# ChrisTho23/DrakeGPT

Hardware: AMD Instinct MI355X
Metric: training tokens/sec (fwd+bwd+AdamW) (higher is better)
Workload: dtype bf16; 1 GPU; TransformerLM_scaled: V=80 C=384 T=256 heads=6 layers=6 dropout=0.2; fwd+bwd+AdamW; hipGraph=on; batch_per_gpu=64, global_batch=64, seq_len=256, parallelism=dp1, dp_gradient_buckets=1, params=10800464

## Files before the change

### drakegpt_amd/_lib.py

```python
from __future__ import annotations

import ctypes as C
import os

import torch

_HERE = os.path.dirname(os.path.abspath(__file__))
LIB_PATH = os.path.join(_HERE, "lib", "libdrakegpt_hip.so")

DG_F32 = 0
DG_BF16 = 1
DG_FP8_E4M3 = 2
DG_FP8_E5M2 = 3
DG_F32X3 = 4
ABI_VERSION = 21


class GemmNtArgs(C.Structure):
    _fields_ = [
        ("A", C.c_void_p), ("lda", C.c_int64),
        ("B", C.c_void_p), ("ldb", C.c_int64),
        ("C", C.c_void_p), ("ldc", C.c_int64),
        ("M", C.c_int32), ("N", C.c_int32), ("K", C.c_int32),
        ("in_dtype", C.c_int32), ("out_dtype", C.c_int32),
# ... 81 lines not shown
    "dg_layernorm_bwd": [_vp, _i, _vp, _vp, _vp, _vp, _vp, _vp, _vp, _vp, _i64, _i, _i, _i, _vp],
    "dg_layernorm_bwd_fused": [_vp, _i, _vp, _vp, _vp, _vp, _vp, _vp, _i, _vp, _vp, _i64, _i, _i, _i, _vp, _i, _f, _vp, _u32, _vp, _vp],
    "dg_layernorm_bwd_fused_fp8": [_vp, _i, _vp, _vp, _vp, _vp, _vp, _vp, _i, _vp, _vp, _i64, _i, _i, _i, _vp, _f, _vp, _u32, _vp, _vp, _vp, _vp, _vp, _i, _vp],
    "dg_gemm_nt": [C.POINTER(GemmNtArgs), _vp],
    "dg_gemm_nt_sign_bits_supported": [C.POINTER(GemmNtArgs)],
    "dg_gemm_nt_fp8_out_supported": [C.POINTER(GemmNtArgs)],
    "dg_gemm_nt_colsum_supported": [C.POINTER(GemmNtArgs)],
    "dg_gemm_nt_colsum_rows": [C.POINTER(GemmNtArgs)],
    "dg_gemm_nt_sign_bits_bytes": [_i, _i],
    "dg_fp8_amax": [_vp, _i, _i64, _vp, _i, _vp, _vp],
    "dg_fp8_quantize": [_vp, _i, _vp, _i, _i64, _vp, _i, _vp, _vp, _vp],
    "dg_fp8_quantize_delayed": [_vp, _i, _vp, _i, _i64, _vp, _vp, _vp, _vp],
    "dg_gemm_tn": [_vp, _i64, _vp, _i64, _vp, _i64, _i64, _i, _i, _i, _i, _i, _vp],
    "dg_gemm_tn_grouped": [C.POINTER(TnProblem), _i, _i, _vp, _i64, _vp],
    "dg_gemm_tn_grouped_workspace_bytes": [C.POINTER(TnProblem), _i],
    "dg_reduce_partials": [_vp, _i64, _i, _vp, _i64, _vp],
    "dg_colsum": [_vp, _i64, _i, _vp, _i64, _i, _i, _i, _vp],
    "dg_dropout_bwd_cast": [_vp, _i, _i64, _vp, _i64, _i, _i, _i, _f, _vp, _u32, _vp, _i64, _vp, _i64, _i, _vp],
    "dg_cast": [_vp, _i, _vp, _i, _i64, _vp],
    "dg_transpose_cast": [_vp, _i64, _vp, _i64, _i, _i, _i, _vp],
    "dg_transpose_cast_batched": [_vp, _i, _i, _i, _i, _vp],
    "dg_transpose_u8_batched": [_vp, _i, _i, _vp],
    "dg_attn_keep_bits_bytes": [_i, _i, _i, _i, _i],
    "dg_attn_fwd": [_vp, _vp, _vp, _i, _i, _i, _i, _f, _f, _vp, _u32, _i, _vp, _i64, _vp],
    "dg_attn_bwd": [_vp, _vp, _vp, _vp, _vp, _vp, _i64, _i, _i, _i, _i, _f, _f, _vp, _u32, _i, _vp, _i64, _vp],
    "dg_attn_fp8_out_supported": [_i, _i, _i, _i, _i],
    "dg_attn_fwd_fp8": [_vp, _vp, _vp, _i, _i, _i, _i, _f, _f, _vp, _u32, _i, _vp, _i64, C.POINTER(AttnFp8Out), _vp],
    "dg_attn_bwd_fp8": [_vp, _vp, _vp, _vp, _vp, _vp, _i64, _i, _i, _i, _i, _f, _f, _vp, _u32, _i, _vp, _i64, C.POINTER(AttnFp8Out), _vp],
    "dg_attn_bwd_workspace_bytes": [_i, _i, _i, _i, _i],
    "dg_attn_decode": [_vp, _vp, _i, _i, _i, _i, _i, _f, _i, _vp],
    "dg_cross_entropy": [_vp, _i, _i64, _vp, _vp, _vp, _i64, _i, _f, _vp, _i, _i, _vp],
    "dg_cross_entropy_fp8": [_vp, _i64, _vp, _vp, _vp, _i64, _f, _i, _i, _vp, _i64, _vp],
    "dg_cross_entropy_fused": [_vp, _i64, _vp, _vp, _vp, _i64, _i, _f, _i, _i, _vp, _i64, _i, _vp, _vp, _vp, _f, _vp],
    "dg_reduce_sum": [_vp, _i64, _f, _vp, _vp],
    "dg_softmax_rows": [_vp, _i64, _vp, _i64, _i, _i, _vp],
    "dg_adamw_step": [_vp, _vp, _vp, _vp, _i64, _vp, _vp, _f, _vp, _i, _vp],
    "dg_sumsq_parts": [_i64],
    "dg_sumsq_partials": [_vp, _i64, _vp, _vp],
    "dg_grad_norm_finalize": [_vp, _i, _f, _vp, _vp, _vp],
    "dg_adamw_step_clip": [_vp, _vp, _vp, _vp, _i64, _vp, _vp, _f, _vp, _vp, _i, _vp],
    "dg_block_chain_supported": [_i, _i],
    "dg_block_chain_fwd": [C.POINTER(BlockChainArgs), _vp],
    "dg_l2_warm": [_vp, _i64, _vp],
    "dg_pack_chain_weights": [_vp, _i64, _vp, _i, _i, _vp],
    "dg_pack_chain_weights_batched": [_vp, _i, _i, _vp],
    "dg_block_chain_bwd_supported": [_i, _i],
    "dg_block_chain_bwd": [C.POINTER(BlockChainBwdArgs), _vp],
}


def _load() -> C.CDLL:
    if not os.path.exists(LIB_PATH):
        raise RuntimeError(
            f"drakegpt_amd: {LIB_PATH} is missing. Build it with `python -m drakegpt_amd.build` "
            "(needs hipcc; cross-compiles for gfx950 without a GPU). There is no CPU fallback.")
    lib = C.CDLL(LIB_PATH)
    for name, argtypes in SIGNATURES.items():
        try:
            fn = getattr(lib, name)
        except AttributeError as e:
            raise RuntimeError(f"drakegpt_amd: {LIB_PATH} does not export {name}; rebuild it") from e
        fn.argtypes = argtypes
        fn.restype = C.c_int
    lib.dg_gemm_nt_sign_bits_bytes.restype = C.c_int64
    lib.dg_gemm_tn_grouped_workspace_bytes.restype = C.c_int64
    lib.dg_attn_bwd_workspace_bytes.restype = C.c_int64
# ... 18 lines not shown
```

### drakegpt_amd/build.py

```python
from __future__ import annotations

import hashlib
import os
import shutil
import subprocess
import sys
from concurrent.futures import ThreadPoolExecutor

PKG = os.path.dirname(os.path.abspath(__file__))
CSRC = os.path.join(PKG, "csrc")
LIBDIR = os.path.join(PKG, "lib")
OBJDIR = os.environ.get("DRAKEGPT_OBJDIR", os.path.join(os.environ.get("TMPDIR", "/tmp"), f"drakegpt_amd_build_{os.getuid()}"))
LIB = os.path.join(LIBDIR, "libdrakegpt_hip.so")
ARCH = "gfx950"

SOURCES = [
    "elementwise.hip",
    "layernorm.hip",
    "gemm.hip",
    "gemm_fp8.hip",
    "gemm_x3.hip",
    "fp8.hip",
    "attention.hip",
    "attention_simple.hip",
    "attention_mfma.hip",
    "cross_entropy.hip",
    "chain.hip",
    "chain_bwd.hip",
    "grad_clip.hip",
]


def _hipcc() -> str:
    for c in (os.environ.get("HIPCC"), "/opt/rocm/bin/hipcc", shutil.which("hipcc")):
        if c and os.path.exists(c):
            return c
    raise RuntimeError("hipcc not found (looked at $HIPCC, /opt/rocm/bin/hipcc, PATH)")


def _digest(paths) -> str:
    h = hashlib.sha256()
    for p in paths:
        with open(p, "rb") as f:
            h.update(f.read())
    return h.hexdigest()


def build(force: bool = False, save_temps: bool = False, verbose: bool = True) -> str:
    os.makedirs(LIBDIR, exist_ok=True)
    os.makedirs(OBJDIR, exist_ok=True)
    hipcc = _hipcc()
    headers = [os.path.join(CSRC, "common.h"), os.path.join(CSRC, "gemm_nt_ws.h"), os.path.join(PKG, "..", "include", "drakegpt_hip.h")]
    hdr_digest = _digest(headers)
    flags = ["--offload-arch=" + ARCH, "-O3", "-fPIC", "-std=c++17",
             "-Wno-unused-result", "-I", os.path.join(PKG, "..", "include")]
    if save_temps:
        flags += ["-save-temps=obj"]

    def compile_one(src: str):
# ... 41 lines not shown
```

### drakegpt_amd/engine.py

```python
from __future__ import annotations

from typing import Dict, List, Optional, Tuple

import torch

from . import ops
from . import sublayers as S
from .model import TransformerLM
from .optim import check_max_grad_norm

Tensor = torch.Tensor
ALIGN = 64


def _round(n: int, a: int = ALIGN) -> int:
    return (n + a - 1) // a * a


class _Layout:
    def __init__(self):
        self.entries: Dict[str, Tuple[int, Tuple[int, ...]]] = {}
        self.size = 0

    def add(self, key: str, shape) -> int:
# ... 178 lines not shown
        self.chain_bwd = (_os.environ.get("DG_CHAIN_BWD", "0") == "1" and self.chain_full and self.stream_dtype == torch.bfloat16
                          and ops.block_chain_bwd_supported(self.M, self.C, self.act))
        self.chain_ln = (_os.environ.get("DG_CHAIN_LN", "0") == "1" and not self.fp8 and self.NH * self.H == self.C
                         and ops.block_chain_supported(self.M, self.C, self.act))
        self._build_layout()
        self.dp_buckets = self._choose_buckets(self._dp_buckets_arg)
        if self.dp_buckets > 1:
            self.chain_bwd = False
        self._alloc_and_adopt()
        self.hyper = torch.tensor([lr, betas[0], betas[1], eps, weight_decay], dtype=torch.float32, device=self.dev)
        self.max_grad_norm = None if max_grad_norm is None else check_max_grad_norm(max_grad_norm)
        self.clip_state = self.norm_work = self.last_grad_norm = None
        if self.max_grad_norm is not None:
            self.clip_state = torch.tensor([0.0, 1.0, self.max_grad_norm, 0.0], dtype=torch.float32, device=self.dev)
            self.norm_work = ops.grad_norm_workspace([self.gflat], self.dev)
            self.last_grad_norm = self.clip_state[0]
        self.state = ops.new_rng_state(seed + 0x9E3779B97F4A7C15 * rank & 0xFFFFFFFFFFFFFFFF, self.dev, 0)
        self.off_block = torch.zeros((self.OFFSET_ROWS, self.B), dtype=torch.int64, device=self.dev)
        self.offsets = self.off_block[0]
        self.off_ctl = torch.tensor([0, 1], dtype=torch.int32, device=self.dev)
        self._off_rows, self._off_left = 1, None
        self.x = torch.zeros((self.B, self.T), dtype=torch.int64, device=self.dev)
        self.y = torch.zeros((self.B, self.T), dtype=torch.int64, device=self.dev)
        self.loss = torch.zeros((), dtype=torch.float32, device=self.dev)
        self.dl_scale = torch.full((1,), 1.0 / (self.M * 57344.0), dtype=torch.float32, device=self.dev)
        self.loss_scratch = torch.zeros((2048 + 1,), dtype=torch.float32, device=self.dev)
        self.corpus: Optional[Tensor] = None
        self._graphs = None
        self._eval_graph = None
        self.force_dp_path = False
        self.debug_timing = False
        self.last_timing: Optional[dict] = None
        self.keep_logits = False
        self.last_logits: Optional[Tensor] = None
        self.refresh_shadows()

    def _build_layout(self):
        C, V, L, NH, H = self.C, self.V, self.L, self.NH, self.H
        A, Bv, E, Z = _Layout(), _Layout(), _Layout(), _Layout()
        for l in range(L):
            A.add(f"{l}.wqkv", (3 * NH * H, C))
            A.add(f"{l}.wproj", (C, NH * H))
            A.add(f"{l}.w1", (4 * C, C))
            A.add(f"{l}.w2", (C, 4 * C))
        A.add("lm.w", (V, C))
        for l in range(L):
            for k, n in (("bproj", C), ("b1", 4 * C), ("b2", C), ("ln1w", C), ("ln1b", C), ("ln2w", C), ("ln2b", C)):
                Bv.add(f"{l}.{k}", (n,))
        Bv.add("lm.b", (V,))
        E.add("tok", (V, C))
        E.add("pos", (self.model.context_length, C))
        Z.add("lnf.w", (C,))
        Z.add("lnf.b", (C,))
        self.layA, self.layB, self.layE, self.layZ = A, Bv, E, Z
        self.offA, self.offB = 0, A.size
        self.offE = A.size + Bv.size
        self.n_active = self.offE + E.size
        self.offZ = self.n_active
        self.n_total = self.n_active + Z.size

    def _choose_buckets(self, arg: Optional[int]) -> int:
        import os
        if arg is None and os.environ.get("DG_DP_BUCKETS"):
            arg = int(os.environ["DG_DP_BUCKETS"])
        if not self.grouped_dw or (self.world == 1 and arg is None):
            return 1
# ... 252 lines not shown
            kw = dict(o=o, x=x, wproj=pk(P["wproj"]), bproj=P["bproj"], ln2w=P["ln2w"], ln2b=P["ln2b"], w1=pk(P["w1"]), b1=P["b1"],
                      w2=pk(P["w2"]), b2=P["b2"], dropout_p=p, rng_state=run.rng, site_proj=S.site_proj(l), site_ffn=S.site_ffn(l))
            if last:
                r = ops.block_chain_fwd(1, M, C, **kw)
            else:
                Pn = self._layer_params(l + 1)
                r = ops.block_chain_fwd(0, M, C, ln1w=Pn["ln1w"], ln1b=Pn["ln1b"], wqkv=pk(Pn["wqkv"]), **kw)
            if want_grad:
                saved.append(((x, h1, m1, r1, qkv, o, lse), (r["x1"], r["h2"], r["mean2"], r["rstd2"], r["f"], r["bits"])))
            x = r["x2"]
            if not last:
                P, h1, m1, r1, qkv = Pn, r["h1"], r["mean1"], r["rstd1"], r["qkv"]
        return x, saved

    def _head(self, run: S.Run, h: Tensor, y_idx: Optional[Tensor], want_grad: bool, saved, M: int):
        if self.bf16_logits and y_idx is not None and not self.keep_logits:
            buf = torch.empty((M, S.k_pad(self.V, self.act)), dtype=self.act, device=self.dev)
            if self.fp8_head and run.fp8 and h.dtype == torch.bfloat16:
                Wl = self.param_view("lm.w")
                xq, xs = S._quantize_operand(run, h, S.E4M3, "lm.x")
                h.dg_fp8x = (xq, xs)
                wq, ws = self.weights.fwd8(Wl)
                logits = ops.gemm_nt(xq, wq, self.act, scale_a=xs, scale_b=ws, bias=self.param_view("lm.b"), out=buf[:, :self.V])
                if want_grad and M == self.M:
                    q8 = torch.empty((M, buf.shape[1]), dtype=S.E5M2, device=self.dev)
                    rows = ops.cross_entropy_fp8(logits, y_idx.view(M), self.V, buf, 1.0 / M, q8)
                    buf.dg_q8 = (q8, self.dl_scale)
                else:
                    rows = ops.cross_entropy(logits, y_idx.view(M), self.V, dlogits=buf if want_grad else None, grad_scale=1.0 / M)
                return None, rows, (saved, h, buf)
            logits, (xa,) = S.linear_fwd(run, h, self.param_view("lm.w"), self.param_view("lm.b"), out=buf[:, :self.V])
            rows = ops.cross_entropy(logits, y_idx.view(M), self.V, dlogits=buf if want_grad else None, grad_scale=1.0 / M)
            return None, rows, (saved, xa, buf)
        logits, (xa,) = S.linear_fwd(run, h, self.param_view("lm.w"), self.param_view("lm.b"), pad_rows=True)
        if y_idx is None:
            return logits, None, None
        dlogits = None
        if want_grad:
            dlogits = torch.empty((M, S.k_pad(self.V, self.act)), dtype=self.act, device=self.dev)
            if M == self.M and ops.cross_entropy_fused_supported(logits, dlogits, self.G):
                part, stride, n = FlatSink(self).vector("lm.b", self.V)
                rows = ops.cross_entropy_fused(logits, y_idx.view(M), self.V, dlogits, 1.0 / M, part, stride, n, self.loss_scratch,
                                               self.loss, 1.0 / M)
                return logits, rows, (saved, xa, dlogits, True)
        rows = ops.cross_entropy(logits, y_idx.view(M), self.V, dlogits=dlogits, grad_scale=1.0 / M)
        return logits, rows, (saved, xa, dlogits)

    def _backward_begin(self, run: S.Run, x_idx: Tensor, ctx) -> dict:
        saved, xa, dlogits = ctx[:3]
        head_done = len(ctx) > 3
        st = dict(run=run, x_idx=x_idx, saved=saved, sink=FlatSink(self), g_next=None, g0=None)
        g = dlogits[:, :self.V]
        q8 = getattr(dlogits, "dg_q8", None)
        if q8 is not None:
            g.dg_fp8 = (q8[0][:, :self.V], q8[1])
        st["dh"] = S.linear_bwd_from_act(run, (xa,), g, self.param_view("lm.w"), True, st["sink"], {"w": "lm.w", "b": "lm.b"},
                                         bias_done=head_done)
        return st

    def _backward_layers(self, st: dict, layers) -> None:
        run, sink, saved, x_idx = st["run"], st["sink"], st["saved"], st["x_idx"]
        B, T = x_idx.shape
        p = self.p_drop
        dh, g_next = st["dh"], st["g_next"]
        for l in layers:
            P = self._layer_params(l)
            sa, sf = saved[l]
            dh, g_next = S.ffn_bwd(run, sf, dh, P["ln2w"], P["w1"], P["w2"], True, p, l, sink,
                                   {"w1": f"{l}.w1", "b1": f"{l}.b1", "w2": f"{l}.w2", "b2": f"{l}.b2", "ln_w": f"{l}.ln2w", "ln_b": f"{l}.ln2b"},
                                   g_in=g_next, emit=(p, S.site_proj(l), f"{l}.bproj", self.C, f"{l}.g_proj"))
            keys = {"wqkv": f"{l}.wqkv", "wproj": f"{l}.wproj", "bproj": f"{l}.bproj", "ln_w": f"{l}.ln1w", "ln_b": f"{l}.ln1b"}
            if l > 0:
                dh, g_next = S.attn_bwd(run, sa, dh, P["ln1w"], P["wqkv"], P["wproj"], True, B, T, self.NH, self.H, p, p, l, sink, keys,
                                        g_in=g_next, emit=(p, S.site_ffn(l - 1), f"{l - 1}.b2", self.C, f"{l - 1}.g_ffn"))
            elif self.onehot is not None:
                dh, st["g0"] = S.attn_bwd(run, sa, dh, P["ln1w"], P["wqkv"], P["wproj"], True, B, T, self.NH, self.H, p, p, l, sink, keys,
                                          g_in=g_next, emit=(0.0, 0, None, self.C))
            elif self.stream_dtype != torch.float32:
                dh, _ = S.attn_bwd(run, sa, dh, P["ln1w"], P["wqkv"], P["wproj"], True, B, T, self.NH, self.H, p, p, l, sink, keys,
                                   g_in=g_next, emit=(0.0, 0, None, self.C))
            else:
                dh = S.attn_bwd(run, sa, dh, P["ln1w"], P["wqkv"], P["wproj"], True, B, T, self.NH, self.H, p, p, l, sink, keys, g_in=g_next)
        st["dh"], st["g_next"] = dh, g_next

# ... 5 lines not shown
        pkT = self.weights.packT
        stride = self.layB.size

        def vec(key, n):
            return sink.vector(key, n)[0]

        def second(l):
            P = self._layer_params(l)
            x1, h2, mean2, rstd2, f, bits = saved[l][1]
            return dict(w2T=pkT(P["w2"]), bits=bits, db1_part=vec(f"{l}.b1", 4 * C), w1T=pkT(P["w1"]), x1=x1, mean2=mean2, rstd2=rstd2,
                        ln2w=P["ln2w"], dln2w_part=vec(f"{l}.ln2w", C), dln2b_part=vec(f"{l}.ln2b", C), gbias2_part=vec(f"{l}.bproj", C),
                        wprojT=pkT(P["wproj"]), site_proj=S.site_proj(l))

        def first(l, dqkv, dresid):
            P = self._layer_params(l)
            x, h1, m1, r1, qkv, o, lse = saved[l][0]
            return dict(dqkv=dqkv, wqkvT=pkT(P["wqkv"]), x=x, mean1=m1, rstd1=r1, ln1w=P["ln1w"], dresid1=dresid,
                        dln1w_part=vec(f"{l}.ln1w", C), dln1b_part=vec(f"{l}.ln1b", C),
                        gbias1_part=vec(f"{l - 1}.b2", C) if l > 0 else None, site_ffn_below=S.site_ffn(l - 1) if l > 0 else 0)

        def weights_and_attention(l, g, r):
            x, h1, m1, r1, qkv, o, lse = saved[l][0]
            x1, h2, mean2, rstd2, f, bits = saved[l][1]
            S.weight_grad(sink, f"{l}.w2", g, f, C, 4 * C)
            S.weight_grad(sink, f"{l}.w1", r["df"], h2, 4 * C, C)
            S.weight_grad(sink, f"{l}.wproj", r["g2"], o, C, C)
            dqkv = ops.attn_bwd(qkv, o, r["dout"], lse, B, T, self.NH, self.H, self.H ** -0.5, p, run.rng, S.site_attn(l))
            S.weight_grad(sink, f"{l}.wqkv", dqkv, h1, 3 * C, C)
            return dqkv

        kw = dict(part_stride=stride, dropout_p=p, rng_state=run.rng)
        dh = st["dh"]
        l = L - 1
        part, pstride, n = sink.vector(f"{l}.b2", C)
        g = ops.dropout_bwd_cast(dh, run.act, p, run.rng, S.site_ffn(l), colsum_part=part, part_stride=pstride, n_partials=n)
        r = ops.block_chain_bwd(1, M, C, g_in=g, dresid2=dh, **second(l), **kw)
        while True:
            dqkv = weights_and_attention(l, g, r)
            if l == 0:
                break
            r = ops.block_chain_bwd(0, M, C, **first(l, dqkv, r["dx2"]), **second(l - 1), **kw)
            g = r["g1"]
            l -= 1
        r = ops.block_chain_bwd(2, M, C, **first(0, dqkv, r["dx2"]), **kw)
        st["dh"], st["g0"], st["g_next"] = r["dx1"], r["g1"], None

    def _backward_end(self, st: dict, group: int = 0) -> None:
        x_idx, dh, sink = st["x_idx"], st["dh"], st["sink"]
        B, T = x_idx.shape
        if self.onehot is not None:
            S.weight_grad(sink, "tok", self.onehot[:, :self.V], st["g0"], self.V, self.C)
            ops.embed_bwd(x_idx, dh.view(B, T, self.C), None, self.grad_view("pos")[:T], V=self.V)
        else:
            ops.embed_bwd(x_idx, dh.view(B, T, self.C), self.grad_view("tok"), self.grad_view("pos")[:T])
        if self.grouped_dw:
            sink.flush(group)
        else:
            ops.reduce_partials(self.slabs, self.layA.size, self.S, self.gflat[self.offA:], self.layA.size)
        ops.reduce_partials(self.vparts, self.layB.size, self.Gv, self.gflat[self.offB:], self.layB.size)

    def _backward(self, run: S.Run, x_idx: Tensor, ctx):
        st = self._backward_begin(run, x_idx, ctx)
        if self.chain_bwd and x_idx.numel() == self.M:
            self._backward_layers_chain(st)
        else:
            self._backward_layers(st, reversed(range(self.L)))
        self._backward_end(st)

# ... 272 lines not shown
```

### drakegpt_amd/ops.py

```python
from __future__ import annotations

import ctypes as C
from typing import Optional

import torch

from . import _lib
from ._lib import DG_BF16, DG_F32, DG_F32X3, DG_FP8_E4M3, DG_FP8_E5M2, GemmNtArgs, check, lib

Tensor = torch.Tensor

_DT = {torch.float32: DG_F32, torch.bfloat16: DG_BF16, torch.float8_e4m3fn: DG_FP8_E4M3, torch.float8_e5m2: DG_FP8_E5M2}
FP8_DTYPES = (torch.float8_e4m3fn, torch.float8_e5m2)
FP8_AMAX_PARTS = 256
ATTN_FP8_HIST = 3 * 64 * 32


def dt_code(dtype: torch.dtype) -> int:
    try:
        return _DT[dtype]
    except KeyError:
        raise TypeError(f"drakegpt_amd: unsupported dtype {dtype} (float32 / bfloat16 / OCP float8 only)") from None


def _stream() -> int:
    return torch.cuda.current_stream().cuda_stream


def _p(t: Optional[Tensor]) -> Optional[int]:
    return None if t is None else t.data_ptr()


def _chk(t: Tensor, name: str, dtype=None, contiguous: bool = True) -> None:
    if not isinstance(t, torch.Tensor) or not t.is_cuda:
        raise RuntimeError(f"drakegpt_amd: {name} must be a tensor on the GPU (got {getattr(t, 'device', type(t))}); "
                           "the HIP path has no CPU fallback")
# ... 590 lines not shown
                                   _p(dlogits_fp8), _ld(dlogits_fp8), _stream()), "dg_cross_entropy_fp8")
    return loss_rows


def cross_entropy_fused_supported(logits: Tensor, dlogits: Tensor, n_partials: int) -> bool:
    return logits.dtype == torch.float32 and _ld(dlogits) <= 128 and 0 < n_partials <= 2048


def cross_entropy_fused(logits: Tensor, targets: Tensor, V: int, dlogits: Tensor, grad_scale: float, colsum_part: Optional[Tensor],
                        part_stride: int, n_partials: int, loss_scratch: Optional[Tensor], loss_out: Optional[Tensor], loss_scale: float,
                        loss_rows: Optional[Tensor] = None) -> Tensor:
    _chk(logits, "logits", torch.float32, contiguous=False)
    _chk(targets, "targets", torch.int64)
    _chk(dlogits, "dlogits", contiguous=False)
    M = logits.shape[0]
    if loss_rows is None:
        loss_rows = torch.empty((M,), dtype=torch.float32, device=logits.device)
    if colsum_part is not None:
        _chk(colsum_part, "colsum_part", torch.float32, contiguous=False)
    cnt = None
    if loss_out is not None:
        _chk(loss_out, "loss_out", torch.float32)
        _chk(loss_scratch, "loss_scratch", torch.float32)
        if loss_scratch.numel() < n_partials + 1:
            raise ValueError("cross_entropy_fused: loss_scratch needs n_partials + 1 words")
        cnt = loss_scratch.data_ptr() + 4 * n_partials
    check(lib.dg_cross_entropy_fused(_p(logits), _ld(logits), _p(targets), _p(loss_rows), _p(dlogits), _ld(dlogits), dt_code(dlogits.dtype),
                                     float(grad_scale), M, V, _p(colsum_part), part_stride, n_partials,
                                     _p(loss_scratch) if loss_out is not None else None, cnt, _p(loss_out), float(loss_scale), _stream()),
          "dg_cross_entropy_fused")
    return loss_rows


def reduce_sum(x: Tensor, scale: float, out: Optional[Tensor] = None) -> Tensor:
    _chk(x, "x", torch.float32)
    if out is None:
        out = torch.empty((), dtype=torch.float32, device=x.device)
    check(lib.dg_reduce_sum(_p(x), x.numel(), float(scale), _p(out), _stream()), "dg_reduce_sum")
    return out


def softmax_rows(logits: Tensor) -> Tensor:
    _chk(logits, "logits", torch.float32, contiguous=False)
    M, V = logits.shape
    probs = torch.empty((M, V), dtype=torch.float32, device=logits.device)
    check(lib.dg_softmax_rows(_p(logits), _ld(logits), _p(probs), V, M, V, _stream()), "dg_softmax_rows")
    return probs


def adamw_step(p: Tensor, g: Tensor, m: Tensor, v: Tensor, hyper: Tensor, rng_state: Tensor, grad_scale: float = 1.0,
               shadow_bf16: Optional[Tensor] = None, n: Optional[int] = None, advance: bool = False, *,
               clip: Optional[Tensor] = None) -> None:
    for t, nm in ((p, "p"), (g, "g"), (m, "m"), (v, "v"), (hyper, "hyper")):
        _chk(t, nm, torch.float32)
    n = p.numel() if n is None else n
    if clip is None:
        check(lib.dg_adamw_step(_p(p), _p(g), _p(m), _p(v), n, _p(hyper), _p(rng_state), float(grad_scale), _p(shadow_bf16), int(advance),
                                _stream()), "dg_adamw_step")
        return
    _chk(clip, "clip", torch.float32)
    check(lib.dg_adamw_step_clip(_p(p), _p(g), _p(m), _p(v), n, _p(hyper), _p(rng_state), float(grad_scale), _p(clip), _p(shadow_bf16),
                                 int(advance), _stream()), "dg_adamw_step_clip")


def grad_norm_workspace(gs, device) -> Tensor:
    return torch.empty(sum(int(lib.dg_sumsq_parts(g.numel())) for g in gs), dtype=torch.float64, device=device)
# ... 173 lines not shown
```

### include/drakegpt_hip.h

```cpp
#ifndef DRAKEGPT_HIP_H
#define DRAKEGPT_HIP_H

#include <stdint.h>

#ifdef __cplusplus
extern "C" {
#endif

#define DG_F32 0
#define DG_BF16 1
#define DG_FP8_E4M3 2
#define DG_FP8_E5M2 3
#define DG_F32X3 4

#define DG_OK 0
#define DG_ERR_ARG (-1)
#define DG_ERR_ALIGN (-2)
#define DG_ERR_DTYPE (-3)

#define DG_ABI_VERSION 21

int dg_version(void);
const char* dg_error_string(int code);

// ... 114 lines not shown
                float scale, float dropout_p, const uint32_t* rng_state, uint32_t site,
                int dtype, void* keep_bits, int64_t keep_bits_bytes, void* stream);
int64_t dg_attn_bwd_workspace_bytes(int B, int T, int NH, int H, int dtype);
int dg_attn_bwd(const void* qkv, const void* out, const void* dout, const float* lse,
                void* dqkv, void* workspace, int64_t workspace_bytes, int B, int T, int NH, int H,
                float scale, float dropout_p, const uint32_t* rng_state, uint32_t site,
                int dtype, const void* keep_bits, int64_t keep_bits_bytes, void* stream);

#define DG_ATTN_FP8_HIST (3 * 64 * 32)
typedef struct dg_attn_fp8_out {
    void* q8; float* hist3; const uint32_t* step_state; float* scale_inv; int only8;
} dg_attn_fp8_out;
int dg_attn_fp8_out_supported(int B, int T, int NH, int H, int dtype);
int dg_attn_fwd_fp8(const void* qkv, void* out, float* lse, int B, int T, int NH, int H,
                    float scale, float dropout_p, const uint32_t* rng_state, uint32_t site,
                    int dtype, void* keep_bits, int64_t keep_bits_bytes, const dg_attn_fp8_out* fp8, void* stream);
int dg_attn_bwd_fp8(const void* qkv, const void* out, const void* dout, const float* lse,
                    void* dqkv, void* workspace, int64_t workspace_bytes, int B, int T, int NH, int H,
                    float scale, float dropout_p, const uint32_t* rng_state, uint32_t site,
                    int dtype, const void* keep_bits, int64_t keep_bits_bytes, const dg_attn_fp8_out* fp8, void* stream);

int dg_attn_decode(const void* qkv_cache, void* out, int B, int Tcap, int t, int NH, int H,
                   float scale, int dtype, void* stream);

int dg_cross_entropy(const void* logits, int logits_dtype, int64_t ldl, const int64_t* targets, float* loss_rows,
                     void* dlogits, int64_t ldd, int dtype, float grad_scale,
                     const float* grad_scale_dev ,
                     int M, int V, void* stream);
int dg_cross_entropy_fp8(const void* logits, int64_t ldl, const int64_t* targets, float* loss_rows, void* dlogits, int64_t ldd,
                         float grad_scale, int M, int V, void* dlogits_fp8, int64_t ld8, void* stream);
int dg_cross_entropy_fused(const float* logits, int64_t ldl, const int64_t* targets, float* loss_rows, void* dlogits, int64_t ldd,
                           int dtype, float grad_scale, int M, int V, float* colsum_part, int64_t part_stride, int n_partials,
                           float* loss_part, uint32_t* loss_counter, float* loss_out, float loss_scale, void* stream);
int dg_reduce_sum(const float* x, int64_t n, float scale, float* out, void* stream);

int dg_softmax_rows(const float* logits, int64_t ldl, float* probs, int64_t ldp, int M, int V,
                    void* stream);

int dg_adamw_step(float* p, const float* g, float* m, float* v, int64_t n, const float* hyper,
                  uint32_t* rng_state, float grad_scale, void* shadow_bf16, int advance_step, void* stream);

int64_t dg_sumsq_parts(int64_t n);
int dg_sumsq_partials(const float* g, int64_t n, double* part, void* stream);
int dg_grad_norm_finalize(const double* part, int n_parts, float grad_scale, const float* max_norm, float* out, void* stream);
int dg_adamw_step_clip(float* p, const float* g, float* m, float* v, int64_t n, const float* hyper, uint32_t* rng_state,
                       float grad_scale, const float* clip_coef, void* shadow_bf16, int advance_step, void* stream);

typedef struct dg_block_chain_args {
    int32_t mode, M, C;
    float eps;
    const void* o; const float* x;
    const void* wproj; const float* bproj; float* x1;
    const float* ln2w; const float* ln2b; float* mean2; float* rstd2; void* h2;
    const void* w1; const float* b1; void* f; uint8_t* sign_bits; int64_t sign_bits_bytes;
    const void* w2; const float* b2; float* x2; void* x2_bf16;
    const float* ln1w; const float* ln1b; float* mean1; float* rstd1; void* h1;
    const void* wqkv; void* qkv;
    float dropout_p; const uint32_t* rng_state; uint32_t site_proj, site_ffn;
} dg_block_chain_args;
int dg_block_chain_supported(int M, int C);
int dg_block_chain_fwd(const dg_block_chain_args* args, void* stream);
int dg_l2_warm(const void* p, int64_t bytes, void* stream);
int dg_pack_chain_weights(const void* w, int64_t ld, void* packed, int N, int K, void* stream);
int dg_pack_chain_weights_batched(const int64_t* desc, int n_desc, int total_stages, void* stream);

typedef struct dg_block_chain_bwd_args {
// ... 21 lines not shown
```

Measured before the change: 7.186 million tokens/s.

## Fuse LM head GEMM, cross-entropy, dlogits backprop and dropout backward into one kernel

Adds a single HIP kernel that computes the LM-head logits with MFMA, the softmax cross-entropy loss and dlogits, the input gradient dh = dlogits·W, and the last FFN dropout backward with the b2 and lm.b bias-gradient column sums. It also does the final loss reduction through a last-block counter. This replaces a chain of separate launches (linear fwd, cross_entropy, dgrad GEMM, dropout_bwd_cast) and avoids writing the fp32 logits to memory and reading them back. The fused path only applies for C=384, V<=128, bf16, and no fp8 or split runs, and it is on by default through engine.fused_head.

```diff
diff --git a/drakegpt_amd/_lib.py b/drakegpt_amd/_lib.py
--- a/drakegpt_amd/_lib.py
+++ b/drakegpt_amd/_lib.py
@@ -137,6 +137,9 @@
     "dg_cross_entropy": [_vp, _i, _i64, _vp, _vp, _vp, _i64, _i, _f, _vp, _i, _i, _vp],
     "dg_cross_entropy_fp8": [_vp, _i64, _vp, _vp, _vp, _i64, _f, _i, _i, _vp, _i64, _vp],
     "dg_cross_entropy_fused": [_vp, _i64, _vp, _vp, _vp, _i64, _i, _f, _i, _i, _vp, _i64, _i, _vp, _vp, _vp, _f, _vp],
+    "dg_loss_head_fused_supported": [_i, _i, _i],
+    "dg_loss_head_fused": [_vp, _i64, _vp, _i64, _vp, _i64, _vp, _vp, _vp, _i64, _vp, _i64, _vp, _i64, _vp, _f, _i, _i, _i, _f, _vp, _u32,
+                           _vp, _vp, _i64, _i, _vp, _vp, _vp, _f, _vp],
     "dg_reduce_sum": [_vp, _i64, _f, _vp, _vp],
     "dg_softmax_rows": [_vp, _i64, _vp, _i64, _i, _i, _vp],
     "dg_adamw_step": [_vp, _vp, _vp, _vp, _i64, _vp, _vp, _f, _vp, _i, _vp],
diff --git a/drakegpt_amd/build.py b/drakegpt_amd/build.py
--- a/drakegpt_amd/build.py
+++ b/drakegpt_amd/build.py
@@ -25,6 +25,7 @@
     "attention_simple.hip",
     "attention_mfma.hip",
     "cross_entropy.hip",
+    "loss_head.hip",
     "chain.hip",
     "chain_bwd.hip",
     "grad_clip.hip",
diff --git a/drakegpt_amd/csrc/loss_head.hip b/drakegpt_amd/csrc/loss_head.hip
--- /dev/null
+++ b/drakegpt_amd/csrc/loss_head.hip
@@ -0,0 +1,328 @@
+#include "common.h"
+
+#define LH_THREADS 256
+#define LH_ROWS 64
+#define LH_C 384
+#define LH_KS1 (LH_C / 32)
+#define LH_NT2 (LH_C / 16 / 4)
+#define LH_DLP 136
+#define LH_GTP (LH_C + 8)
+#define LH_RL 5
+
+struct LhParams {
+    const bf16_t* x; int64_t ldx;
+    const bf16_t* w; int64_t ldw;
+    const bf16_t* wt; int64_t ldwt;
+    const float* bias;
+    const int64_t* targets;
+    bf16_t* dlogits; int64_t ldd;
+    bf16_t* dh; int64_t lddh;
+    bf16_t* g; int64_t ldg;
+    float* loss_rows;
+    float* lmb_part; float* b2_part; int64_t part_stride;
+    int M, V, rows_per;
+    float grad_scale;
+    float inv_keep; uint32_t thr; int drop; const uint32_t* rng_state; uint32_t site;
+    float* loss_part; unsigned* counter; float* loss_out; float loss_scale;
+};
+
+template <int NJ>
+__global__ __launch_bounds__(LH_THREADS) void loss_head_fused_kernel(LhParams p) {
+    constexpr int KS2 = (NJ + 1) / 2;
+    constexpr int GT_BYTES = LH_ROWS * LH_GTP * 2, RED_BYTES = LH_ROWS * 128 * 4, W_BYTES = NJ * 16 * LH_GTP * 2;
+    constexpr int U_BYTES = W_BYTES > GT_BYTES + RED_BYTES ? W_BYTES : GT_BYTES + RED_BYTES;
+    __shared__ __attribute__((aligned(16))) bf16_t dl[LH_ROWS * LH_DLP];
+    __shared__ __attribute__((aligned(16))) char ubuf[U_BYTES];
+    bf16_t* const wl = (bf16_t*)ubuf;
+    bf16_t* const gt = (bf16_t*)ubuf;
+    float (*const red)[128] = (float (*)[128])(ubuf + GT_BYTES);
+    __shared__ float lred[LH_ROWS];
+    __shared__ unsigned last_flag;
+    const int tid = threadIdx.x, lane = tid & 63, wave = tid >> 6;
+    const int fr = lane & 15, fg = lane >> 4;
+    const int V = p.V;
+    const int m_begin = blockIdx.x * p.rows_per;
+    int m_end = m_begin + p.rows_per; if (m_end > p.M) m_end = p.M;
+
+    u32x4 wtf[LH_NT2][KS2];
+    float bj[NJ];
+#pragma unroll
+    for (int j = 0; j < NJ; ++j) {
+        int n = j * 16 + fr; if (n > V - 1) n = V - 1;
+        bj[j] = p.bias[n];
+    }
+    uint32_t key = 0;
+    if (p.drop) key = dg_site_key_dev(p.rng_state, p.site);
+
+    const int crl = tid / (LH_C / 8), cch = (tid - crl * (LH_C / 8)) * 8;
+    float cacc[4][NJ], lsum[4], cs[8];
+#pragma unroll
+    for (int e = 0; e < 4; ++e) {
+        lsum[e] = 0.f;
+#pragma unroll
+        for (int j = 0; j < NJ; ++j) cacc[e][j] = 0.f;
+    }
+#pragma unroll
+    for (int e = 0; e < 8; ++e) cs[e] = 0.f;
+
+    for (int r0 = m_begin; r0 < m_end; r0 += LH_ROWS) {
+        const int mrow = r0 + wave * 16;
+        {
+            int ar = mrow + fr; if (ar > p.M - 1) ar = p.M - 1;
+            const bf16_t* xp = p.x + (int64_t)ar * p.ldx + fg * 8;
+            u32x4 xa[LH_KS1];
+#pragma unroll
+            for (int s = 0; s < LH_KS1; ++s) xa[s] = *(const u32x4*)(xp + s * 32);
+            constexpr int WCH = NJ * 16 * (LH_C / 8);
+            u32x4 wst[(WCH + LH_THREADS - 1) / LH_THREADS];
+#pragma unroll
+            for (int i = 0; i < (WCH + LH_THREADS - 1) / LH_THREADS; ++i) {
+                const int id = tid + LH_THREADS * i, r = id / (LH_C / 8), c = id - r * (LH_C / 8);
+                if (id < WCH) wst[i] = *(const u32x4*)(p.w + (int64_t)(r < V ? r : V - 1) * p.ldw + c * 8);
+            }
+            int64_t tg[4];
+#pragma unroll
+            for (int e = 0; e < 4; ++e) {
+                const int row = mrow + fg * 4 + e;
+                tg[e] = p.targets[row < m_end ? row : p.M - 1];
+            }
+#pragma unroll
+            for (int i = 0; i < (WCH + LH_THREADS - 1) / LH_THREADS; ++i) {
+                const int id = tid + LH_THREADS * i, r = id / (LH_C / 8), c = id - r * (LH_C / 8);
+                if (id < WCH) *(u32x4*)(wl + r * LH_GTP + c * 8) = wst[i];
+            }
+            __syncthreads();
+            f32x4 acc[NJ];
+#pragma unroll
+            for (int j = 0; j < NJ; ++j) acc[j] = (f32x4){0.f, 0.f, 0.f, 0.f};
+            u32x4 wb[2][NJ];
+#pragma unroll
+            for (int j = 0; j < NJ; ++j) wb[0][j] = *(const u32x4*)(wl + (j * 16 + fr) * LH_GTP + fg * 8);
+#pragma unroll
+            for (int s = 0; s < LH_KS1; ++s) {
+                if (s + 1 < LH_KS1) {
+#pragma unroll
+                    for (int j = 0; j < NJ; ++j) wb[(s + 1) & 1][j] = *(const u32x4*)(wl + (j * 16 + fr) * LH_GTP + (s + 1) * 32 + fg * 8);
+                }
+#pragma unroll
+                for (int j = 0; j < NJ; ++j)
+                    acc[j] = __builtin_amdgcn_mfma_f32_16x16x32_bf16(__builtin_bit_cast(bf16x8, xa[s]), __builtin_bit_cast(bf16x8, wb[s & 1][j]), acc[j], 0, 0, 0);
+            }
+#pragma unroll
+            for (int nt = 0; nt < LH_NT2; ++nt)
+#pragma unroll
+                for (int ks = 0; ks < KS2; ++ks)
+                    wtf[nt][ks] = *(const u32x4*)(p.wt + (int64_t)((wave * LH_NT2 + nt) * 16 + fr) * p.ldwt + ks * 32 + fg * 8);
+#pragma unroll
+            for (int e = 0; e < 4; ++e) {
+                const int rl = wave * 16 + fg * 4 + e;
+                const int row = r0 + rl;
+                const bool ok = row < m_end;
+                float v[NJ];
+                float mx = -INFINITY;
+#pragma unroll
+                for (int j = 0; j < NJ; ++j) {
+                    v[j] = (j * 16 + fr) < V ? acc[j][e] + bj[j] : -INFINITY;
+                    mx = fmaxf(mx, v[j]);
+                }
+#pragma unroll
+                for (int o = 8; o > 0; o >>= 1) mx = fmaxf(mx, __shfl_xor(mx, o, 64));
+                int64_t t = tg[e];
+                t = t < 0 ? 0 : (t >= V ? V - 1 : t);
+                float xc = 0.f;
+#pragma unroll
+                for (int j = 0; j < NJ; ++j) xc = j == (int)(t >> 4) ? v[j] : xc;
+                const float xt = __shfl(xc, (lane & 48) | (int)(t & 15), 64);
+                float s = 0.f;
+#pragma unroll
+                for (int j = 0; j < NJ; ++j) { v[j] = expf(v[j] - mx); s += v[j]; }
+#pragma unroll
+                for (int o = 8; o > 0; o >>= 1) s += __shfl_xor(s, o, 64);
+                const float lr = mx + logf(s) - xt;
+                if (ok && fr == 0) {
+                    if (p.loss_rows) p.loss_rows[row] = lr;
+                    lsum[e] += lr;
+                }
+                const float inv = 1.f / s;
+#pragma unroll
+                for (int j = 0; j < NJ; ++j) {
+                    const int i = j * 16 + fr;
+                    const float gk = i < V ? (v[j] * inv - (i == (int)t ? 1.f : 0.f)) * p.grad_scale : 0.f;
+                    if (ok) cacc[e][j] += gk;
+                    dl[rl * LH_DLP + i] = (bf16_t)gk;
+                }
+#pragma unroll
+                for (int j = NJ; j < 8; ++j) dl[rl * LH_DLP + j * 16 + fr] = (bf16_t)0.f;
+            }
+        }
+        __syncthreads();
+        {
+            const int cpr = (int)(p.ldd >> 3);
+            for (int id = lane; id < 16 * cpr; id += 64) {
+                const int rr = id / cpr, c16 = id - rr * cpr;
+                const int row = mrow + rr;
+                if (row < m_end) *(u32x4*)(p.dlogits + (int64_t)row * p.ldd + c16 * 8) = *(const u32x4*)(dl + (wave * 16 + rr) * LH_DLP + c16 * 8);
+            }
+        }
+#pragma unroll 2
+        for (int mt = 0; mt < LH_ROWS / 16; ++mt) {
+            f32x4 a2[LH_NT2];
+#pragma unroll
+            for (int nt = 0; nt < LH_NT2; ++nt) a2[nt] = (f32x4){0.f, 0.f, 0.f, 0.f};
+#pragma unroll
+            for (int ks = 0; ks < KS2; ++ks) {
+                const u32x4 df = *(const u32x4*)(dl + (mt * 16 + fr) * LH_DLP + ks * 32 + fg * 8);
+#pragma unroll
+                for (int nt = 0; nt < LH_NT2; ++nt)
+                    a2[nt] = __builtin_amdgcn_mfma_f32_16x16x32_bf16(__builtin_bit_cast(bf16x8, wtf[nt][ks]), __builtin_bit_cast(bf16x8, df), a2[nt], 0, 0, 0);
+            }
+            const int row = r0 + mt * 16 + fr;
+            const bool ok = row < m_end;
+#pragma unroll
+            for (int nt = 0; nt < LH_NT2; ++nt) {
+                const int col = wave * (LH_NT2 * 16) + nt * 16 + fg * 4;
+                float v[4];
+                bf16x4 o, kept;
+#pragma unroll
+                for (int e = 0; e < 4; ++e) { o[e] = (bf16_t)a2[nt][e]; v[e] = (float)o[e]; }
+                kept = o;
+                if (p.drop) {
+                    const uint32_t w2 = (((uint32_t)row * (uint32_t)LH_C + (uint32_t)col) >> 1) * DG_WEYL;
+#pragma unroll
+                    for (int e = 0; e < 4; e += 2) {
+                        const uint32_t h = dg_hash_w(key, w2 + (uint32_t)(e >> 1) * DG_WEYL);
+                        const bool k0 = dg_keep_lo(h, p.thr), k1 = dg_keep_hi(h, p.thr);
+                        v[e] = k0 ? v[e] * p.inv_keep : 0.f;
+                        v[e + 1] = k1 ? v[e + 1] * p.inv_keep : 0.f;
+                        kept[e] = k0 ? o[e] : (bf16_t)0.f;
+                        kept[e + 1] = k1 ? o[e + 1] : (bf16_t)0.f;
+                    }
+                }
+                if (ok) {
+                    *(bf16x4*)(p.dh + (int64_t)row * p.lddh + col) = o;
+                    bf16x4 go;
+#pragma unroll
+                    for (int e = 0; e < 4; ++e) go[e] = (bf16_t)v[e];
+                    *(bf16x4*)(p.g + (int64_t)row * p.ldg + col) = go;
+                }
+                *(bf16x4*)(gt + (mt * 16 + fr) * LH_GTP + col) = kept;
+            }
+        }
+        __syncthreads();
+        if (p.b2_part && crl < LH_RL) {
+            const int nrows = m_end - r0 < LH_ROWS ? m_end - r0 : LH_ROWS;
+            int r = crl - (r0 - m_begin) % LH_RL; if (r < 0) r += LH_RL;
+#pragma unroll 4
+            for (; r < nrows; r += LH_RL) {
+                const bf16x8 tv = *(const bf16x8*)(gt + r * LH_GTP + cch);
+#pragma unroll
+                for (int e = 0; e < 8; ++e) {
+                    float x = (float)tv[e];
+                    if (p.drop) x *= p.inv_keep;
+                    cs[e] += x;
+                }
+            }
+        }
+        __syncthreads();
+    }
+
+#pragma unroll
+    for (int e = 0; e < 4; ++e)
+        if (fr == 0) lred[wave * 16 + fg * 4 + e] = lsum[e];
+    float* r5 = &red[0][0];
+    if (p.b2_part && crl < LH_RL) {
+#pragma unroll
+        for (int e = 0; e < 8; ++e) r5[crl * LH_C + cch + e] = cs[e];
+    }
+    __syncthreads();
+    if (p.loss_out && tid == 0) {
+        float b = 0.f;
+#pragma unroll 8
+        for (int r = 0; r < LH_ROWS; ++r) b += lred[r];
+        __hip_atomic_store(p.loss_part + blockIdx.x, b, __ATOMIC_RELAXED, __HIP_MEMORY_SCOPE_AGENT);
+    }
+    if (p.b2_part) {
+        for (int c = tid; c < LH_C; c += LH_THREADS) {
+            float x = 0.f;
+#pragma unroll
+            for (int k = 0; k < LH_RL; ++k) x += r5[k * LH_C + c];
+            p.b2_part[(int64_t)blockIdx.x * p.part_stride + c] = x;
+        }
+    }
+    __syncthreads();
+#pragma unroll
+    for (int e = 0; e < 4; ++e) {
+        const int rl = wave * 16 + fg * 4 + e;
+#pragma unroll
+        for (int j = 0; j < NJ; ++j) red[rl][j * 16 + fr] = cacc[e][j];
+    }
+    __syncthreads();
+    if (p.lmb_part && tid < V) {
+        float c = 0.f;
+#pragma unroll 8
+        for (int r = 0; r < LH_ROWS; ++r) c += red[r][tid];
+        p.lmb_part[(int64_t)blockIdx.x * p.part_stride + tid] = c;
+    }
+    if (!p.loss_out) return;
+    if (tid == 0) {
+        asm volatile("s_waitcnt vmcnt(0)" ::: "memory");
+        const unsigned prev = __hip_atomic_fetch_add(p.counter, 1u, __ATOMIC_RELAXED, __HIP_MEMORY_SCOPE_AGENT);
+        last_flag = prev == gridDim.x - 1 ? 1u : 0u;
+    }
+    __syncthreads();
+    if (!last_flag) return;
+    __builtin_amdgcn_fence(__ATOMIC_ACQUIRE, "workgroup");
+    float* sh = &red[0][0];
+    for (int i = tid; i < (int)gridDim.x; i += LH_THREADS) sh[i] = __hip_atomic_load(p.loss_part + i, __ATOMIC_RELAXED, __HIP_MEMORY_SCOPE_AGENT);
+    __syncthreads();
+    if (tid == 0) {
+        float tot = 0.f;
+        int i = 0;
+        for (; i + 8 <= (int)gridDim.x; i += 8) {
+            const f32x4 a = *(const f32x4*)(sh + i), b = *(const f32x4*)(sh + i + 4);
+            tot += a[0]; tot += a[1]; tot += a[2]; tot += a[3]; tot += b[0]; tot += b[1]; tot += b[2]; tot += b[3];
+        }
+        for (; i < (int)gridDim.x; ++i) tot += sh[i];
+        p.loss_out[0] = tot * p.loss_scale;
+        __hip_atomic_store(p.counter, 0u, __ATOMIC_RELAXED, __HIP_MEMORY_SCOPE_AGENT);
+    }
+}
+
+extern "C" int dg_loss_head_fused_supported(int M, int C, int V) { return M > 0 && C == LH_C && V > 0 && V <= 128 ? 1 : 0; }
+
+extern "C" int dg_loss_head_fused(const void* x, int64_t ldx, const void* w, int64_t ldw, const void* wt, int64_t ldwt, const float* bias,
+                                  const int64_t* targets, void* dlogits, int64_t ldd, void* dh, int64_t lddh, void* g, int64_t ldg,
+                                  float* loss_rows, float grad_scale, int M, int C, int V, float p, const uint32_t* rng_state, uint32_t site,
+                                  float* lmb_part, float* b2_part, int64_t part_stride, int n_partials,
+                                  float* loss_part, uint32_t* loss_counter, float* loss_out, float loss_scale, void* stream) {
+    if (!x || !w || !wt || !bias || !targets || !dlogits || !dh || !g) return DG_ERR_ARG;
+    if (!dg_loss_head_fused_supported(M, C, V)) return DG_ERR_ARG;
+    const int nj = (V + 15) / 16, ks2 = (nj + 1) / 2;
+    if (ldx < C || ldw < C || lddh < C || ldg < C || ldd < V || ldd > 128 || ldwt < 32 * ks2) return DG_ERR_ARG;
+    if (n_partials <= 0 || n_partials > 2048 || p < 0.f || p >= 1.f) return DG_ERR_ARG;
+    if ((lmb_part && part_stride < V) || (b2_part && part_stride < C)) return DG_ERR_ARG;
+    if ((loss_out != nullptr) != (loss_part != nullptr) || (loss_out != nullptr) != (loss_counter != nullptr)) return DG_ERR_ARG;
+    if (ldx % 8 || ldw % 8 || ldwt % 8 || ldd % 8 || lddh % 8 || ldg % 8 || !dg_aligned16(x) || !dg_aligned16(w) || !dg_aligned16(wt) ||
+        !dg_aligned16(dlogits) || !dg_aligned16(dh) || !dg_aligned16(g))
+        return DG_ERR_ALIGN;
+    LhParams q;
+    q.x = (const bf16_t*)x; q.ldx = ldx; q.w = (const bf16_t*)w; q.ldw = ldw; q.wt = (const bf16_t*)wt; q.ldwt = ldwt;
+    q.bias = bias; q.targets = targets;
+    q.dlogits = (bf16_t*)dlogits; q.ldd = ldd; q.dh = (bf16_t*)dh; q.lddh = lddh; q.g = (bf16_t*)g; q.ldg = ldg;
+    q.loss_rows = loss_rows; q.lmb_part = lmb_part; q.b2_part = b2_part; q.part_stride = part_stride;
+    q.M = M; q.V = V; q.rows_per = (M + n_partials - 1) / n_partials;
+    q.grad_scale = grad_scale;
+    q.drop = (p > 0.f && rng_state) ? 1 : 0;
+    q.inv_keep = 1.f / (1.f - p); q.thr = dg_drop_threshold(p); q.rng_state = rng_state; q.site = site;
+    q.loss_part = loss_part; q.counter = (unsigned*)loss_counter; q.loss_out = loss_out; q.loss_scale = loss_scale;
+    const dim3 grid(n_partials), block(LH_THREADS);
+    hipStream_t s = (hipStream_t)stream;
+    switch (nj) {
+#define LH_CASE(N) case N: hipLaunchKernelGGL(loss_head_fused_kernel<N>, grid, block, 0, s, q); break
+        LH_CASE(1); LH_CASE(2); LH_CASE(3); LH_CASE(4); LH_CASE(5); LH_CASE(6); LH_CASE(7); LH_CASE(8);
+#undef LH_CASE
+        default: return DG_ERR_ARG;
+    }
+    DG_LAUNCH_CHECK();
+    return DG_OK;
+}
diff --git a/drakegpt_amd/engine.py b/drakegpt_amd/engine.py
--- a/drakegpt_amd/engine.py
+++ b/drakegpt_amd/engine.py
@@ -234,6 +234,7 @@
         self.debug_timing = False
         self.last_timing: Optional[dict] = None
         self.keep_logits = False
+        self.fused_head = True
         self.last_logits: Optional[Tensor] = None
         self.refresh_shadows()
 
@@ -552,6 +553,16 @@
             logits, (xa,) = S.linear_fwd(run, h, self.param_view("lm.w"), self.param_view("lm.b"), out=buf[:, :self.V])
             rows = ops.cross_entropy(logits, y_idx.view(M), self.V, dlogits=buf if want_grad else None, grad_scale=1.0 / M)
             return None, rows, (saved, xa, buf)
+        if want_grad and y_idx is not None and M == self.M and self._fused_head_ok(run, h):
+            Wl = self.param_view("lm.w")
+            dlogits = torch.empty((M, S.k_pad(self.V, self.act)), dtype=self.act, device=self.dev)
+            sink = FlatSink(self)
+            lmb, stride, n = sink.vector("lm.b", self.V)
+            b2 = sink.vector(f"{self.L - 1}.b2", self.C)[0]
+            dh, g = ops.loss_head_fused(h, self.weights.fwd(Wl), self.weights.bwd(Wl), self.param_view("lm.b"), y_idx.view(M), dlogits,
+                                        1.0 / M, run.p(self.p_drop), run.rng, S.site_ffn(self.L - 1), lmb, b2, stride, n,
+                                        self.loss_scratch, self.loss, 1.0 / M)
+            return None, None, (saved, h, dlogits, True, dh, g)
         logits, (xa,) = S.linear_fwd(run, h, self.param_view("lm.w"), self.param_view("lm.b"), pad_rows=True)
         if y_idx is None:
             return logits, None, None
@@ -566,10 +577,19 @@
         rows = ops.cross_entropy(logits, y_idx.view(M), self.V, dlogits=dlogits, grad_scale=1.0 / M)
         return logits, rows, (saved, xa, dlogits)
 
+    def _fused_head_ok(self, run: S.Run, h: Tensor) -> bool:
+        return (self.fused_head and not self.keep_logits and not self.bf16_logits and self.act == torch.bfloat16 and h.dtype == torch.bfloat16
+                and not run.fp8 and not run.split and run.stream == torch.bfloat16 and 0 < self.G <= 2048
+                and ops.loss_head_fused_supported(self.M, self.C, self.V))
+
     def _backward_begin(self, run: S.Run, x_idx: Tensor, ctx) -> dict:
         saved, xa, dlogits = ctx[:3]
         head_done = len(ctx) > 3
         st = dict(run=run, x_idx=x_idx, saved=saved, sink=FlatSink(self), g_next=None, g0=None)
+        if len(ctx) > 4:
+            S.weight_grad(st["sink"], "lm.w", dlogits[:, :self.V], xa, self.V, self.C)
+            st["dh"], st["g_next"] = ctx[4], ctx[5]
+            return st
         g = dlogits[:, :self.V]
         q8 = getattr(dlogits, "dg_q8", None)
         if q8 is not None:
@@ -641,8 +661,10 @@
         kw = dict(part_stride=stride, dropout_p=p, rng_state=run.rng)
         dh = st["dh"]
         l = L - 1
-        part, pstride, n = sink.vector(f"{l}.b2", C)
-        g = ops.dropout_bwd_cast(dh, run.act, p, run.rng, S.site_ffn(l), colsum_part=part, part_stride=pstride, n_partials=n)
+        g = st["g_next"]
+        if g is None:
+            part, pstride, n = sink.vector(f"{l}.b2", C)
+            g = ops.dropout_bwd_cast(dh, run.act, p, run.rng, S.site_ffn(l), colsum_part=part, part_stride=pstride, n_partials=n)
         r = ops.block_chain_bwd(1, M, C, g_in=g, dresid2=dh, **second(l), **kw)
         while True:
             dqkv = weights_and_attention(l, g, r)
diff --git a/drakegpt_amd/ops.py b/drakegpt_amd/ops.py
--- a/drakegpt_amd/ops.py
+++ b/drakegpt_amd/ops.py
@@ -1,7 +1,7 @@
 from __future__ import annotations
 
 import ctypes as C
-from typing import Optional
+from typing import Optional, Tuple
 
 import torch
 
@@ -658,6 +658,42 @@
     return loss_rows
 
 
+def loss_head_fused_supported(M: int, C: int, V: int) -> bool:
+    return bool(lib.dg_loss_head_fused_supported(M, C, V))
+
+
+def loss_head_fused(x: Tensor, w: Tensor, wt: Tensor, bias: Tensor, targets: Tensor, dlogits: Tensor, grad_scale: float, p: float,
+                    rng_state: Optional[Tensor], site: int, lmb_part: Optional[Tensor], b2_part: Optional[Tensor], part_stride: int,
+                    n_partials: int, loss_scratch: Optional[Tensor], loss_out: Optional[Tensor], loss_scale: float,
+                    loss_rows: Optional[Tensor] = None) -> Tuple[Tensor, Tensor]:
+    for t, name in ((x, "x"), (w, "w"), (wt, "wt"), (dlogits, "dlogits")):
+        _chk(t, name, torch.bfloat16, contiguous=False)
+    _chk(bias, "bias", torch.float32)
+    _chk(targets, "targets", torch.int64)
+    M, Cc = x.shape
+    V = w.shape[0]
+    if w.shape[1] != Cc or wt.shape[0] != Cc or bias.numel() != V or targets.numel() != M or dlogits.shape[0] != M:
+        raise ValueError("loss_head_fused: shapes do not agree")
+    dh = torch.empty((M, Cc), dtype=torch.bfloat16, device=x.device)
+    g = torch.empty((M, Cc), dtype=torch.bfloat16, device=x.device)
+    for t, name in ((lmb_part, "lmb_part"), (b2_part, "b2_part"), (loss_rows, "loss_rows")):
+        if t is not None:
+            _chk(t, name, torch.float32, contiguous=False)
+    cnt = None
+    if loss_out is not None:
+        _chk(loss_out, "loss_out", torch.float32)
+        _chk(loss_scratch, "loss_scratch", torch.float32)
+        if loss_scratch.numel() < n_partials + 1:
+            raise ValueError("loss_head_fused: loss_scratch needs n_partials + 1 words")
+        cnt = loss_scratch.data_ptr() + 4 * n_partials
+    check(lib.dg_loss_head_fused(_p(x), _ld(x), _p(w), _ld(w), _p(wt), _ld(wt), _p(bias), _p(targets), _p(dlogits), _ld(dlogits),
+                                 _p(dh), Cc, _p(g), Cc, _p(loss_rows), float(grad_scale), M, Cc, V, float(p),
+                                 _p(rng_state) if p > 0.0 else None, site, _p(lmb_part), _p(b2_part), part_stride, n_partials,
+                                 _p(loss_scratch) if loss_out is not None else None, cnt, _p(loss_out), float(loss_scale), _stream()),
+          "dg_loss_head_fused")
+    return dh, g
+
+
 def reduce_sum(x: Tensor, scale: float, out: Optional[Tensor] = None) -> Tensor:
     _chk(x, "x", torch.float32)
     if out is None:
diff --git a/include/drakegpt_hip.h b/include/drakegpt_hip.h
--- a/include/drakegpt_hip.h
+++ b/include/drakegpt_hip.h
@@ -170,6 +170,12 @@
 int dg_cross_entropy_fused(const float* logits, int64_t ldl, const int64_t* targets, float* loss_rows, void* dlogits, int64_t ldd,
                            int dtype, float grad_scale, int M, int V, float* colsum_part, int64_t part_stride, int n_partials,
                            float* loss_part, uint32_t* loss_counter, float* loss_out, float loss_scale, void* stream);
+int dg_loss_head_fused_supported(int M, int C, int V);
+int dg_loss_head_fused(const void* x, int64_t ldx, const void* w, int64_t ldw, const void* wt, int64_t ldwt, const float* bias,
+                       const int64_t* targets, void* dlogits, int64_t ldd, void* dh, int64_t lddh, void* g, int64_t ldg,
+                       float* loss_rows, float grad_scale, int M, int C, int V, float p, const uint32_t* rng_state, uint32_t site,
+                       float* lmb_part, float* b2_part, int64_t part_stride, int n_partials,
+                       float* loss_part, uint32_t* loss_counter, float* loss_out, float loss_scale, void* stream);
 int dg_reduce_sum(const float* x, int64_t n, float scale, float* out, void* stream);
 
 int dg_softmax_rows(const float* logits, int64_t ldl, float* probs, int64_t ldp, int M, int V,
```

Result: no change. 7.186 million tokens/s (-0.0%).
